# TAdeJong/pyGPA

Hardware: AMD Instinct MI355X
Metric: Mpixels/s displacement-field extraction (3 peaks, 4096^2 img) + achieved HBM GB/s (higher is better)
Workload: dtype f32; 1 GPU; 4096x4096 synthetic hex moire, 3 Bragg peaks x 16 k-vectors, sigma=10, weighted DCT-PCG unwrap kmax=10, image resident in HBM, u downloaded to pinned host memory inside the step (BASELINE.json configs[2]); x_planes=12, d2h_of_u=included, overlapped with the next step (copy stream), images_in_flight=1

## Files before the change

### pygpa_amd/csrc/gpa_api.hip

```cpp
#include "gpa_plan.h"

static thread_local std::string g_err;
int gpa_fail(int code, const std::string& msg) {
  g_err = msg;
  return code;
}
namespace gpa {
static const char* const kOptNames[OPT_COUNT] = {
    "PBS_FULLBAND", "SERIAL_UNWRAP", "NO_WORKER", "NO_KSPLIT", "NO_COMPACT", "NO_SHARED",
    "NO_PAIR", "PBS_E8", "TRI_SMALL", "TRI_Q", "NO_MR", "MR_FORCE_BLUESTEIN", "NO_ROWPQ", "COLSOLVE", "NO_LAT",
    "F32_EPS_FLOOR", "COLSTREAM_CHUNK", "NO_ROWHALF", "PAIR_MAXSIDE", "ROWHALF_MINLG", "NO_PQDCT",
    "NO_REORDER", "NO_RAW", "NO_TILEFUSE", "NO_ROWPERS", "NO_LFTILE", "LF_ALL_ROUNDS", "DFT_ENGINE", "GAUSS_FFT_MINR", "NO_GAUSS2D", "NO_DFT_HALF", "F32_STALL", "PBS_LDS_PAD", "NO_SHARED_PHASES", "PA_STAG", "PA_STAG_TICKS", "PA_ROT"};
static OptVal g_opts[OPT_COUNT];
static std::once_flag g_opts_once;
static void opt_assign(OptVal& o, const char* value) {
  o.set = value != nullptr;
  o.num = value ? atof(value) : 0.0;
  memset(o.str, 0, sizeof(o.str));
  if (value) strncpy(o.str, value, sizeof(o.str) - 1);
}
static void opts_from_env() {
  for (int k = 0; k < OPT_COUNT; ++k) opt_assign(g_opts[k], getenv((std::string("GPA_") + kOptNames[k]).c_str()));
}
const OptVal& opt(OptKey k) {
  std::call_once(g_opts_once, opts_from_env);
  return g_opts[k];
}
}

Axis make_axis(int n) {
  Axis a;
  a.n = n;
  int lg = 0;
  while ((1 << lg) < n) ++lg;
  if ((1 << lg) == n) {
    a.padded = false;
  } else {
    lg = 0;
    while ((1 << lg) < 2 * n - 1) ++lg;
    a.padded = true;
  }
  if (lg < 6) {
    lg = 6;
    a.padded = ((1 << lg) != n);
  }
  a.lg = lg;
  a.L = 1 << lg;
  a.extL = a.padded ? n - 1 : 0;
  a.extR = 0;
  return a;
}

Axis compact_axis(const Axis& full, int E) {
  if (!full.padded || E >= (full.n - 1) / 2) return full;
  int lg = 6;
  while ((1 << lg) < full.n + 2 * E) ++lg;
  if (lg >= full.lg) return full;
  Axis a = full;
  a.lg = lg;
  a.L = 1 << lg;
  a.extL = a.extR = E;
  return a;
}

int upload_real_table(gpa_plan* p, void* dst, const std::vector<double>& v) {
  if (p->dtype == GPA_F32) HIP_TRY(upload_as<float>(dst, v, p->stream));
  else HIP_TRY(upload_as<double>(dst, v, p->stream));
  return GPA_OK;
}

int dmalloc(gpa_plan* p, void** ptr, size_t bytes) {
  if (bytes == 0) bytes = 16;
  hipError_t e = hipMalloc(ptr, bytes);
  if (e != hipSuccess)
    return fail(GPA_ERR_HIP, std::string("hipMalloc(") + std::to_string(bytes) + "): " + hipGetErrorString(e));
  p->ws_bytes += bytes;
  return GPA_OK;
}
int plan_build(gpa_plan* p) {
  HIP_TRY(hipSetDevice(p->device));
  HIP_TRY(hipStreamCreateWithFlags(&p->stream, hipStreamNonBlocking));
  HIP_TRY(hipEventCreate(&p->ev0));
  HIP_TRY(hipEventCreate(&p->ev1));
  for (auto& e : p->stage_ev) HIP_TRY(hipEventCreate(&e));
  const size_t npx = (size_t)p->n0 * p->n1;
  const int B = p->max_batch;
  for (int ax = 0; ax < 2; ++ax) {
    const Axis& a = ax == 0 ? p->ax0 : p->ax1;
    std::vector<double> t((size_t)2 * a.L);
    for (int k = 0; k < a.L; ++k) {
      t[2 * k] = cos(-2.0 * M_PI * k / a.L);
      t[2 * k + 1] = sin(-2.0 * M_PI * k / a.L);
    }
    void** dst = ax == 0 ? &p->tw0 : &p->tw1;
    TRY(dmalloc(p, dst, (size_t)a.L * p->csz));
    TRY(upload_real_table(p, *dst, t));
  }
  TRY(dmalloc(p, &p->Hx, (size_t)p->ax0.L * p->csz));
  TRY(dmalloc(p, &p->Hy, (size_t)p->ax1.L * p->csz));
  p->tbuf_planes = B < 4 ? B : 4;
  TRY(dmalloc(p, &p->Tbuf, (size_t)p->tbuf_planes * npx * p->csz));
  TRY(dmalloc(p, &p->tb.cxb, (size_t)B * std::max(p->ax0.L / 16, 256) * p->csz));
  TRY(dmalloc(p, &p->tb.sx, (size_t)B * 16 * p->csz));
  TRY(dmalloc(p, &p->tb.wxw, (size_t)B * p->csz));
  TRY(dmalloc(p, &p->tb.wxr, (size_t)B * p->csz));
  TRY(dmalloc(p, &p->tb.cyb, (size_t)B * std::max(p->ax1.L / 16, 256) * p->csz));
  TRY(dmalloc(p, &p->tb.sy, (size_t)B * 16 * p->csz));
  TRY(dmalloc(p, &p->tb.wyw, (size_t)B * p->csz));
  TRY(dmalloc(p, &p->tb.wyr, (size_t)B * p->csz));
  TRY(dmalloc(p, (void**)&p->tb.planeof, (size_t)B * sizeof(int)));
  TRY(dmalloc(p, (void**)&p->d_pw, (size_t)B * sizeof(double)));
  TRY(dmalloc(p, &p->tb.dx, (size_t)B * p->n0 * p->csz));
  TRY(dmalloc(p, &p->tb.dy, (size_t)B * p->n1 * p->csz));
  TRY(dmalloc(p, (void**)&p->d_kl, (size_t)B * 2 * sizeof(double)));
  TRY(dmalloc(p, (void**)&p->d_kr, (size_t)B * 2 * sizeof(double)));
  HIP_TRY(hipHostMalloc((void**)&p->h_k, ((size_t)B * 6 + 32) * sizeof(double)));
  HIP_TRY(hipHostMalloc((void**)&p->h_iters, 8 * sizeof(int)));
  TRY(dmalloc(p, &p->d_image, npx * p->rsz));
  TRY(dmalloc(p, &p->d_mean, 16));
  TRY(dmalloc(p, &p->d_tile_mean, 16));
  TRY(dmalloc(p, (void**)&p->d_scratch, 16384 * sizeof(double)));
  TRY(dmalloc(p, &p->d_aux0, (size_t)p->n0 * 2 * sizeof(double)));
  TRY(dmalloc(p, &p->d_aux1, (size_t)p->n1 * 2 * sizeof(double)));
  p->max_peaks = B < 8 ? B : 8;
  TRY(dmalloc(p, &p->d_lockin, (size_t)p->max_peaks * npx * p->csz));
  TRY(dmalloc(p, (void**)&p->d_kidx, (size_t)p->max_peaks * npx * sizeof(int32_t)));
  TRY(dmalloc(p, &p->d_dudx, 2 * npx * p->rsz));
  TRY(dmalloc(p, &p->d_dudy, 2 * npx * p->rsz));
  TRY(dmalloc(p, &p->d_wnorm, npx * p->rsz));
  TRY(dmalloc(p, &p->d_u, 2 * npx * p->rsz));
  TRY(dmalloc(p, (void**)&p->d_kmat, (size_t)p->max_peaks * 2 * sizeof(double)));
  if (!p->spectral_only) {
    size_t before = 0;
    hipError_t e = unwrap_workspace_create(p->dtype, p->n0, p->n1, p->stream, &p->uw, &before);
    if (e != hipSuccess) return fail(GPA_ERR_HIP, std::string("unwrap workspace: ") + hipGetErrorString(e));
    p->ws_bytes += before;
  }
  return GPA_OK;
}


int upload_twiddles(gpa_plan* p, void* dst, int L) {
  std::vector<double> t((size_t)2 * L);
  for (int k = 0; k < L; ++k) {
    t[2 * k] = cos(-2.0 * M_PI * k / L);
    t[2 * k + 1] = sin(-2.0 * M_PI * k / L);
  }
  return upload_real_table(p, dst, t);
}

extern "C" {

int gpa_version(void) { return 100; }

int gpa_set_option(const char* name, const char* value) {
  if (!name) return fail(GPA_ERR_ARG, "gpa_set_option: null name");
  if (strncmp(name, "GPA_", 4) == 0) name += 4;
  (void)opt(OPT_NO_LAT);
  for (int k = 0; k < OPT_COUNT; ++k)
    if (strcmp(name, kOptNames[k]) == 0) {
      opt_assign(g_opts[k], value);
      return GPA_OK;
    }
  return fail(GPA_ERR_ARG, std::string("gpa_set_option: unknown option ") + name);
}
// ... 177 lines not shown
```

### pygpa_amd/csrc/gpa_internal.h

```cpp
#pragma once
#include <hip/hip_runtime.h>
#include <stdint.h>

#include "gpa_fft.h"
#include "gpa_mrfft.h"

namespace gpa {

struct KernelProfiler {
  struct Rec { const char* name; hipEvent_t a, b; };
  static constexpr int MAXREC = 4096;
  Rec rec[MAXREC];
  int n = 0;
  hipEvent_t pool[2 * MAXREC];
  int npool = 0;
};
extern thread_local KernelProfiler* g_kprof;
struct ProfScope {
  hipStream_t s;
  KernelProfiler::Rec* r = nullptr;
  ProfScope(const char* name, hipStream_t stream) : s(stream) {
    KernelProfiler* k = g_kprof;
    if (!k || k->n >= KernelProfiler::MAXREC) return;
    for (int j = 0; j < 2; ++j)
      if (k->npool < 2 * (k->n + 1)) { if (hipEventCreate(&k->pool[k->npool]) != hipSuccess) return; ++k->npool; }
    r = &k->rec[k->n];
    r->name = name;
    r->a = k->pool[2 * k->n];
    r->b = k->pool[2 * k->n + 1];
    ++k->n;
    (void)hipEventRecord(r->a, s);
  }
  ~ProfScope() { if (r) (void)hipEventRecord(r->b, s); }
};
#if defined(__HIPCC__)
__device__ __forceinline__ int xcd_tile(int b, int grid) {
  const int base = grid >> 3, rem = grid & 7, x = b & 7, idx = b >> 3;
  return x * base + (x < rem ? x : rem) + idx;
}
#endif

inline hipError_t set_dynamic_lds_once(const void* kern, int bytes, unsigned& done) {
  int dev = 0;
  (void)hipGetDevice(&dev);
  const unsigned bit = 1u << (dev & 31);
  if (done & bit) return hipSuccess;
  hipError_t e = hipFuncSetAttribute(kern, hipFuncAttributeMaxDynamicSharedMemorySize, bytes);
  if (e == hipSuccess) done |= bit;
  return e;
}

inline int device_cus() {
  static int n[32] = {};
  int dev = 0;
  (void)hipGetDevice(&dev);
  int& slot = n[dev & 31];
  if (!slot) {
    int cus = 0;
    if (hipDeviceGetAttribute(&cus, hipDeviceAttributeMultiprocessorCount, dev) != hipSuccess || cus <= 0) cus = 256;
    slot = cus;
  }
  return slot;
}

enum OptKey {
  OPT_PBS_FULLBAND, OPT_SERIAL_UNWRAP, OPT_NO_WORKER, OPT_NO_KSPLIT, OPT_NO_COMPACT, OPT_NO_SHARED,
  OPT_NO_PAIR, OPT_PBS_E8, OPT_TRI_SMALL, OPT_TRI_Q, OPT_NO_MR, OPT_MR_FORCE_BLUESTEIN, OPT_NO_ROWPQ,
  OPT_COLSOLVE, OPT_NO_LAT, OPT_F32_EPS_FLOOR, OPT_COLSTREAM_CHUNK, OPT_NO_ROWHALF, OPT_PAIR_MAXSIDE, OPT_ROWHALF_MINLG, OPT_NO_PQDCT,
  OPT_NO_REORDER, OPT_NO_RAW, OPT_NO_TILEFUSE, OPT_NO_ROWPERS, OPT_NO_LFTILE, OPT_LF_ALL_ROUNDS, OPT_DFT_ENGINE, OPT_GAUSS_FFT_MINR, OPT_NO_GAUSS2D, OPT_NO_DFT_HALF, OPT_F32_STALL, OPT_PBS_LDS_PAD, OPT_NO_SHARED_PHASES, OPT_PA_STAG, OPT_PA_STAG_TICKS, OPT_PA_ROT, OPT_COUNT
};
struct OptVal {
  bool set;
  double num;
  char str[24];
};
const OptVal& opt(OptKey k);
inline bool opt_set(OptKey k) { return opt(k).set; }

#define GPA_PROF_CAT2(a, b) a##b
#define GPA_PROF_CAT(a, b) GPA_PROF_CAT2(a, b)
#define GPA_PROF(name, stream) ::gpa::ProfScope GPA_PROF_CAT(_gpa_prof_, __LINE__)(name, stream)

struct Axis {
  int n;
  int lg;
  int L;
  bool padded;
  int extL, extR;
};
inline int axis_tpf(const Axis& a) { return a.L / 16; }

GPA_HD int axis_src(int m, int n, int L, bool padded, int extL, int extR) {
  if (!padded) return m;
  if (m < n) return m;
  if (m < n + extR) return m - n;
  if (m >= L - extL) return m - L + n;
  return -1;
}

struct SweepTables {
  void* cxb;
  void* sx;
  void* wxw;
  void* wxr;
  void* cyb;
  void* sy;
  void* wyw;
  void* wyr;
  void* dx;
  void* dy;
  int* planeof;
};

hipError_t launch_tables(int dtype, const Axis& a0, const Axis& a1, const double* kl,
                         const double* kr, int B, const double* pw, int Bx, const SweepTables& tb,
                         hipStream_t s);
hipError_t launch_mean(int dtype, const void* image, size_t count, double* scratch,
                       void* mean_out, hipStream_t s, int nimg = 1);
hipError_t launch_passA(int dtype, const Axis& a0, int n1, const void* image, const void* mean,
                        const SweepTables& tb, const void* Hx, const void* tw0, void* Tbuf,
                        int Bx, hipStream_t s, int nimg = 1);
hipError_t launch_passB(int dtype, const Axis& a1, int n0, const void* Tbuf, const void* Hy,
                        const void* tw1, const SweepTables& tb, int P, int K, bool select,
                        void* out, int32_t* kidx, hipStream_t s, int nimg = 1, int Bx = 0);
hipError_t launch_passB_ext(int dtype, const Axis& a1, int n0, const void* Tbuf, const void* Hy, const void* tw1,
                            const SweepTables& tb, int K, int mode, void* out, int32_t* kidx, const uint8_t* gate,
                            void* psi, hipStream_t s, int P = 1);
hipError_t launch_passB_split(int dtype, const Axis& a1, int n0, const void* Tbuf, const void* Hy, const void* tw1,
                              const SweepTables& tb, int P, int K, int ksplit, void* part, int32_t* pidx, void* out,
                              int32_t* kidx, hipStream_t s);
hipError_t launch_phasegrad(int dtype, const void* psi, int K, const int32_t* kidx, int n0, int n1, const double* kl,
                            const double* kr, int mode, void* grad, hipStream_t s, const double* ystep = nullptr, int P = 1);
int passA_cols(int dtype, int lg);
int spec_index_rt(int lg, int tid, int reg, int elems = 16);

hipError_t launch_reconstruct(int dtype, const void* lockin, const double* kmat ,
                              int P, int n0, int n1, int border, void* dudx, void* dudy,
                              void* wnorm, hipStream_t s, const double* ystep = nullptr );

hipError_t launch_reconstruct_tile(int dtype, const void* lockin, const double* kmat, int P, int n0, int n1, int border,
                                   int i0, int j0, int t0, int t1, void* const dx[2], size_t dx_pitch, void* const dy[2],
                                   size_t dy_pitch, void* const wn[2], size_t wn_pitch, hipStream_t s,
                                   const double* ystep = nullptr);
hipError_t launch_reconstruct_setup(int dtype, const void* lockin, const double* kmat, int P, int n0, int n1,
                                    int border, void* wnorm, void* r0, void* r1, double* part0, double* part1,
                                    int* nparts, hipStream_t s, int nimg = 1, size_t rstride = 0, size_t pstride = 0,
                                    const double* ystep = nullptr );

hipError_t launch_prediff(int dtype, const void* grads, const void* w, const double* kmat, int P, int n0, int n1,
                          void* dudx, void* dudy, void* wnorm, hipStream_t s);

hipError_t launch_wlstsq(int dtype, const void* b, const void* w, const double* kmat, int P, size_t npx,
                         void* out, hipStream_t s);

hipError_t launch_jacobian(int dtype, const void* grads, const void* w, const double* kmat, int P, size_t npx,
                           double nmperpixel, const double* dks , void* J, hipStream_t s);
hipError_t launch_cabs(int dtype, const void* z, size_t count, void* out, hipStream_t s);
hipError_t launch_props(int dtype, const void* jac, size_t npx, int add_identity, double refangle, double refscale,
                        int diff, void* out, hipStream_t s);

int huber_sums_offset();
hipError_t launch_huber_moments(int dtype, const void* img, int n0, int n1, const double* coef, double cx, double cy,
                                double sx, double sy, double* scratch, hipStream_t s);

constexpr int PEAK_PARTS = 1024;
bool gauss2d_small_ok(int R);
hipError_t launch_gauss2d_small(int dtype, const void* in, void* out, int n0, int n1, const double* w, int R,
                                const void* minuend, hipStream_t s);
hipError_t launch_gauss1d(int dtype, const void* in, void* out, int n0, int n1, int axis, const double* w, int R,
                          const void* minuend, hipStream_t s);
hipError_t launch_localmax(int dtype, const void* smooth, int n0, int n1, double rel, double* part, double* thr,
                           int max_out, int* count, int32_t* coords, void* vals, hipStream_t s);

hipError_t launch_deconv_pack(int dtype, const void* data, int m0, int m1, int pad, void* Z, hipStream_t s);
hipError_t launch_deconv_filter(int dtype, void* Z, int n0, int n1, const double* gx, const double* gy, double balance,
                                hipStream_t s);
hipError_t launch_deconv_unpack(int dtype, const void* Z, int m0, int m1, int pad, void* out, hipStream_t s);

hipError_t launch_tile_sums(int dtype, const void* wins, size_t win_stride, size_t pitch, const int* rects_dev, int ntiles,
                            int max_rows, double* part, double* out, hipStream_t s);
int tile_sums_bands(int max_rows);
hipError_t launch_set_mean(int dtype, const double* sum, double scale, void* mean_out, hipStream_t s);
hipError_t launch_copy_fields(int dtype, const void* const* src, void* const* dst, const size_t* src_pitch,
                              const size_t* dst_pitch, const int* rows, const int* cols, int nf, hipStream_t s);
hipError_t launch_stitch(int dtype, const void* tiles, size_t slot_stride, size_t field_stride, size_t tile_pitch,
                         const int* table_dev, int ntiles, int t0, int t1, int nf, void* const* dst, const size_t* dst_pitch,
                         const int* dst_rows, const int* dst_cols, hipStream_t s);

struct WarpWs {
  void* buf = nullptr;
  size_t cap = 0;
  void* taps = nullptr;
  int taps_dtype = -1;
  size_t* counted = nullptr;
};
void warp_ws_free(WarpWs* ws);
hipError_t warp_reserve_undistort(int dtype, int n0, int n1, WarpWs* ws, hipStream_t s);
hipError_t warp_invert_u(int dtype, const void* d_u, int n0, int n1, double scale, int iters, int edge, int shift,
                         void* d_out, hipStream_t s, int mode, int nan_last, WarpWs* ws, const int* rects = nullptr, int nrect = 0);
hipError_t warp_image(int dtype, const void* d_img, const void* d_uinv, int n0, int n1, void* d_out, hipStream_t s, WarpWs* ws,
                      const int* rects = nullptr, int nrect = 0);
hipError_t spline_coef_constant_f64(const double* d_in, int n0, int n1, double* d_tmp, double* d_out, hipStream_t s, WarpWs* ws);

struct UcellGeom {
  double ks[4], kinv[4], rmin[2], z;
  int rs0, rs1;
};
struct UcellWs {
  void* buf = nullptr;
  size_t cap = 0;
  WarpWs spline{};
  void* stage = nullptr;
  size_t stage_cap = 0;
  size_t* counted = nullptr;
};
void ucell_ws_free(UcellWs* ws);
hipError_t ucell_stage(UcellWs* ws, size_t bytes, hipStream_t s, void** out);
constexpr int UCELL_MAX_FRAMES = 65535;
constexpr long long UCELL_MAX_BINS = 1LL << 24;
hipError_t ucell_average(int dtype, const void* d_images, int B, const void* d_u, int n0, int n1, const UcellGeom& g,
                         double* d_res, double* d_weights, hipStream_t s, UcellWs* ws);
hipError_t ucell_expand(int dtype, const double* d_cell, const UcellGeom& g, double z2, const void* d_u, int n0, int n1,
// ... 4 lines not shown
```

### pygpa_amd/csrc/gpa_passb_shared.hip

```cpp
#include <stdlib.h>

#include "gpa_internal.h"
#include "gpa_passb_shared.h"

namespace gpa {

template <class T> struct MfmaVec;
template <> struct MfmaVec<float> { typedef float type __attribute__((ext_vector_type(4))); };
template <> struct MfmaVec<double> { typedef double type __attribute__((ext_vector_type(4))); };

__device__ __forceinline__ MfmaVec<float>::type mfma16(float a, float b, MfmaVec<float>::type c) {
  return __builtin_amdgcn_mfma_f32_16x16x4f32(a, b, c, 0, 0, 0);
}
__device__ __forceinline__ MfmaVec<double>::type mfma16(double a, double b, MfmaVec<double>::type c) {
  return __builtin_amdgcn_mfma_f64_16x16x4f64(a, b, c, 0, 0, 0);
}
template <class T> __device__ __forceinline__ int mfma_row(int kq, int r) {
  if constexpr (sizeof(T) == 8) return kq + 4 * r;
  else return 4 * kq + r;
}

template <class T> struct upair { T u, v; };

#ifndef GPA_PBS_NOFIX
#define GPA_PBS_NOFIX 0
#endif
#ifndef GPA_PBS_EXECSTORE
#define GPA_PBS_EXECSTORE 0
#endif
#ifndef GPA_PBS_NOSTORE
#define GPA_PBS_NOSTORE 0
#endif
#ifndef GPA_PBS_WAVESKIP
#define GPA_PBS_WAVESKIP 1
#endif
#ifndef GPA_PBS_NTLOAD
#define GPA_PBS_NTLOAD 1
#endif

template <class T, int TPF, int EE>
__device__ __forceinline__ void load_gb(T (&h)[EE], const T* gbrow, int tid) {
  using gscalar = const __attribute__((address_space(1))) T;
  gscalar* gb = (gscalar*)gbrow;
#pragma unroll
  for (int i = 0; i < EE; ++i) h[i] = gb[i * TPF + tid];
}
template <class T> __device__ __forceinline__ cpx<T> load_cpx(__amdgpu_buffer_rsrc_t r, int voff, int soff, int aux = 16);
__device__ __forceinline__ cpx<float> load_once(const cpx<float>* p) {
  typedef float v2f_t __attribute__((ext_vector_type(2)));
  const v2f_t d = __builtin_nontemporal_load(reinterpret_cast<const v2f_t*>(p));
  return {d.x, d.y};
}
__device__ __forceinline__ cpx<double> load_once(const cpx<double>* p) {
  typedef double v2d_t __attribute__((ext_vector_type(2)));
  const v2d_t d = __builtin_nontemporal_load(reinterpret_cast<const v2d_t*>(p));
  return {d.x, d.y};
}

typedef int v2i_t __attribute__((ext_vector_type(2)));
typedef int v4i_t __attribute__((ext_vector_type(4)));
__device__ __forceinline__ void store_cpx(cpx<double> v, __amdgpu_buffer_rsrc_t r, int voff, int soff);
__device__ __forceinline__ void store_cpx(cpx<float> v, __amdgpu_buffer_rsrc_t r, int voff, int soff) {
  v2i_t d = {__float_as_int(v.x), __float_as_int(v.y)};
  __builtin_amdgcn_raw_buffer_store_b64(d, r, voff, soff, 0);
}
template <> __device__ __forceinline__ cpx<float> load_cpx<float>(__amdgpu_buffer_rsrc_t r, int voff, int soff, int aux) {
  v2i_t d = aux == 16 ? __builtin_amdgcn_raw_buffer_load_b64(r, voff, soff, 16) : aux == 2 ? __builtin_amdgcn_raw_buffer_load_b64(r, voff, soff, 2) : __builtin_amdgcn_raw_buffer_load_b64(r, voff, soff, 0);
  return {__int_as_float(d.x), __int_as_float(d.y)};
}
template <> __device__ __forceinline__ cpx<double> load_cpx<double>(__amdgpu_buffer_rsrc_t r, int voff, int soff, int aux) {
  v4i_t d = aux == 16 ? __builtin_amdgcn_raw_buffer_load_b128(r, voff, soff, 16) : aux == 2 ? __builtin_amdgcn_raw_buffer_load_b128(r, voff, soff, 2) : __builtin_amdgcn_raw_buffer_load_b128(r, voff, soff, 0);
  const long long a = ((long long)(unsigned)d.x) | ((long long)d.y << 32), b = ((long long)(unsigned)d.z) | ((long long)d.w << 32);
  return {__longlong_as_double(a), __longlong_as_double(b)};
}
__device__ __forceinline__ void store_pair(cpx<float> a, cpx<float> b, __amdgpu_buffer_rsrc_t r, int voff, int soff) {
  v4i_t d = {__float_as_int(a.x), __float_as_int(a.y), __float_as_int(b.x), __float_as_int(b.y)};
  __builtin_amdgcn_raw_buffer_store_b128(d, r, voff, soff, 0);
}
__device__ __forceinline__ void store_pair(cpx<double> a, cpx<double> b, __amdgpu_buffer_rsrc_t r, int voff, int soff) {
  store_cpx(a, r, voff, soff);
  store_cpx(b, r, voff + 16, soff);
}
__device__ __forceinline__ void store_cpx(cpx<double> v, __amdgpu_buffer_rsrc_t r, int voff, int soff) {
  const long long a = __double_as_longlong(v.x), b = __double_as_longlong(v.y);
  v4i_t d = {(int)a, (int)(a >> 32), (int)b, (int)(b >> 32)};
  __builtin_amdgcn_raw_buffer_store_b128(d, r, voff, soff, 0);
}

template <class T, int LG, int EE = 16>
struct PassBSGeom {
  using F = WgFFT<T, LG, EE>;
  static_assert(F::P == 3 || F::P == 4, "three- or four-pass transforms");
  static constexpr int TPF = F::TPF;
  static_assert(TPF >= 64, "a row needs whole wavefronts");
#ifndef GPA_PBS_MINTHREADS
#define GPA_PBS_MINTHREADS 128
#endif
  static constexpr int NF = TPF >= GPA_PBS_MINTHREADS ? 1 : GPA_PBS_MINTHREADS / TPF;
  static constexpr int THREADS = NF * TPF;
  static constexpr int NW = TPF / 64;
  static constexpr int NC = PassBSharedNC<T>::value;
  static constexpr int LOGNC = NC == 4 ? 2 : 1;
  static constexpr bool STAGE = sizeof(T) == 4;
#ifndef GPA_PBS_TWL
#define GPA_PBS_TWL 1
#endif
  static constexpr bool TWL = GPA_PBS_TWL && F::P == 3;
  static constexpr int T1 = TWL ? F::P1_SETS * 6 : 0;
  static constexpr int SV = sizeof(T) == 4 ? 4 : 2;
  __host__ __device__ static size_t row_elems(int Epad) {
    const size_t ES = (size_t)Epad + 4;
    return (size_t)F::LDS_ELEMS + SV * ES + 2 * NC * ES + (STAGE ? 3 * NC * ES : 0);
  }
  __host__ __device__ static size_t lds_bytes(int Epad) {
    return (NF * row_elems(Epad) + T1) * sizeof(cpx<T>) + (2 * (size_t)Epad + 16) * sizeof(T);
  }
};

#ifndef GPA_PBS_F32_WAVES
#define GPA_PBS_F32_WAVES 3
#endif
#ifndef GPA_PBS_PAD_WAVES
#define GPA_PBS_PAD_WAVES 3
#endif
#ifndef GPA_PBS_F64_WAVES
#define GPA_PBS_F64_WAVES 2
#endif

#ifndef GPA_PBS_E8_WAVES
#define GPA_PBS_E8_WAVES 4
#endif
#ifndef GPA_PBS_E8_F64_WAVES
#define GPA_PBS_E8_F64_WAVES 2
#endif
#ifndef GPA_PBS_L13_WAVES
#define GPA_PBS_L13_WAVES 3
#endif
template <class T, int LG, bool PADDED, int EE, int NBL, bool PSI = false>
__global__ __launch_bounds__((PassBSGeom<T, LG, EE>::THREADS),
                             (EE == 8 ? (sizeof(T) == 8 ? GPA_PBS_E8_F64_WAVES : GPA_PBS_E8_WAVES)
                                      : (sizeof(T) == 8 ? GPA_PBS_F64_WAVES : (LG >= 13 ? GPA_PBS_L13_WAVES : (PADDED ? GPA_PBS_PAD_WAVES : GPA_PBS_F32_WAVES))))) void passB_shared_kernel(
    const cpx<T>* __restrict__ Tin, int n0, int n1, const T* __restrict__ Gb, const cpx<T>* __restrict__ twtab,
    const int* __restrict__ planeof, const int* __restrict__ order, const int* __restrict__ desc, const cpx<T>* __restrict__ pre_g,
    const cpx<T>* __restrict__ psi, const T* __restrict__ gtab, const cpx<T>* __restrict__ dx,
    const cpx<T>* __restrict__ dyc, const cpx<T>* __restrict__ rot16, int K, int E, int Epad, cpx<T>* out,
    int32_t* kidx, int P, int Bx, int raw, T* __restrict__ psi_out) {
  using F = WgFFT<T, LG, EE>;
  using G = PassBSGeom<T, LG, EE>;
  using V4 = typename MfmaVec<T>::type;
  constexpr int TPF = F::TPF, L = F::L, NC = G::NC;
  constexpr bool STAGE = G::STAGE;
  extern __shared__ __attribute__((aligned(16))) char smem[];
  const int tid = threadIdx.x % TPF, f = __builtin_amdgcn_readfirstlane(threadIdx.x / TPF);
  cpx<T>* lds = reinterpret_cast<cpx<T>*>(smem) + (size_t)f * G::row_elems(Epad);
  upair<T>* strip = reinterpret_cast<upair<T>*>(lds + F::LDS_ELEMS);
  const int ES = Epad + 4;
  cpx<T>* fixb = lds + F::LDS_ELEMS + G::SV * ES;
  cpx<T>* pre_l = fixb + 2 * NC * ES;
  cpx<T>* psi_l = pre_l + NC * ES;
  cpx<T>* t1 = reinterpret_cast<cpx<T>*>(smem) + (size_t)G::NF * G::row_elems(Epad);
  T* glds = reinterpret_cast<T*>(t1 + G::T1);
  const int row = blockIdx.x * G::NF + f;
  const bool valid = row < n0;
  const int rr = valid ? row : 0;
  const int p = blockIdx.y, pt = p % P, img = p / P;
  const int lane = threadIdx.x & 63, wrow = tid >> 6;

  for (int i = threadIdx.x; i < 2 * Epad + 16; i += G::THREADS) glds[i] = gtab[i];
#ifndef GPA_PBS_TWREG_F32
#define GPA_PBS_TWREG_F32 1
#endif
  constexpr bool TWLK = G::TWL && !(GPA_PBS_TWREG_F32 && sizeof(T) == 4 && !PADDED);
  typename std::conditional<TWLK, typename F::TwiddlesP1Lds, typename F::Twiddles>::type tw;
  if constexpr (TWLK) {
    F::fill_pass1_table(t1, twtab, threadIdx.x, G::THREADS);
    __syncthreads();
    F::load_twiddles(tw, twtab, tid, t1);
  } else {
    F::load_twiddles(tw, twtab, tid);
  }

  T ab[EE];
#pragma unroll
  for (int i = 0; i < EE; ++i) ab[i] = T(0);
  const size_t obase = ((size_t)p * n0 + rr) * n1;
  const __amdgpu_buffer_rsrc_t orow = __builtin_amdgcn_make_buffer_rsrc((void*)(out + obase), 0, n1 * (int)sizeof(cpx<T>), 0x00020000);
  const __amdgpu_buffer_rsrc_t krow = __builtin_amdgcn_make_buffer_rsrc((void*)(kidx ? kidx + obase : nullptr), 0, kidx ? n1 * 4 : 0, 0x00020000);
  constexpr int OOB = (int)0x80000000;
  const int iA = PADDED ? (n1 - E) / TPF : EE - 1, iB = PADDED ? (n1 - 1) / TPF : EE - 1;

  cpx<T> X[NBL];
  T h[NBL];
  const cpx<T> rot = rot16[pt * EE + (tid & (EE - 1))];
  const cpx<T> rot_tail = rot16[pt * EE + ((n1 - 1 - (tid < E ? tid : 0)) & (EE - 1))];
#ifndef GPA_PBS_PREFETCH_F64
#define GPA_PBS_PREFETCH_F64 0
#endif
#ifndef GPA_PBS_PREFETCH_F32
#define GPA_PBS_PREFETCH_F32 1
#endif
  constexpr bool PREFETCH = NBL < EE && (sizeof(T) == 8 ? GPA_PBS_PREFETCH_F64 : GPA_PBS_PREFETCH_F32);
  for (int k = 0; k < K; ++k) {
    const int b = pt * K + k;
    const int ob = order[b];
    const int d = desc[b];
    if (d & 1) {
      const cpx<T>* src = Tin + (((size_t)img * Bx + planeof[ob]) * n0 + rr) * n1;
      const cpx<T> cs0 = dx[(size_t)ob * n0 + rr];
      const cpx<T> cs = cmul(cs0, rot);
      cpx<T> tail = {T(0), T(0)};
      if (tid < E) tail = src[n1 - 1 - tid];
      cpx<T> XX[EE];
      if constexpr (PADDED) {
        const __amdgpu_buffer_rsrc_t srow = __builtin_amdgcn_make_buffer_rsrc((void*)src, 0, n1 * (int)sizeof(cpx<T>), 0x00020000);
#pragma unroll
        for (int i = 0; i < EE; ++i)
          XX[i] = cmul(load_cpx<T>(srow, (tid + TPF * i) * (int)sizeof(cpx<T>), 0, GPA_PBS_NTLOAD ? 2 : 0), cs);
      } else {
#pragma unroll
        for (int i = 0; i < EE; ++i) XX[i] = cmul(GPA_PBS_NTLOAD ? load_once(src + tid + TPF * i) : src[tid + TPF * i], cs);
      }
      if (tid < Epad) {
        const bool in = tid < E;
        const cpx<T> s0 = in ? XX[0] : cpx<T>{T(0), T(0)};
        const cpx<T> s1 = in ? cmul(tail, cmul(cs0, rot_tail)) : cpx<T>{T(0), T(0)};
        if constexpr (G::SV == 4) {
          strip[0 * ES + tid] = {s0.x, -s0.y};
          strip[1 * ES + tid] = {s0.y, s0.x};
          strip[2 * ES + tid] = {s1.x, s1.y};
          strip[3 * ES + tid] = {s1.y, -s1.x};
        } else {
          strip[0 * ES + tid] = {s0.x, s0.y};
          strip[1 * ES + tid] = {s1.x, s1.y};
        }
      }
      F::forward(XX, lds, tid, tw);
#pragma unroll
      for (int i = 0; i < NBL; ++i) X[i] = XX[i];
    }
    const int par = (d >> 7) & 1;
    cpx<T> y[EE];
    {
      if (!PREFETCH || k == 0) load_gb<T, TPF, NBL>(h, Gb + (size_t)b * (NBL * TPF), tid);
      if constexpr (STAGE) {
        if (d & 2) {
          const int nc = (d >> 4) & 7;
          for (int e = tid; e < NC * Epad; e += TPF) {
            const int c = e / Epad, j = e - c * Epad, cc = c < nc ? c : nc - 1;
            pre_l[c * ES + j] = pre_g[(size_t)(b + cc) * Epad + j];
            psi_l[(par * NC + c) * ES + j] = psi[(size_t)(b + cc) * Epad + j];
          }
        }
      }
#pragma unroll
      for (int i = 0; i < EE; ++i) {
        if (i < NBL) y[i] = {X[i < NBL ? i : 0].x * h[i < NBL ? i : 0], X[i < NBL ? i : 0].y * h[i < NBL ? i : 0]};
        else y[i] = {T(0), T(0)};
      }
    }
    cpx<T> psL = {T(0), T(0)}, psR = {T(0), T(0)};
    const int a0R = PADDED ? 0 : TPF - 1 - tid;
    if constexpr (!STAGE) {
      psL = psi[(size_t)b * Epad + (tid < E ? tid : 0)];
      psR = psi[(size_t)b * Epad + (a0R < E ? a0R : 0)];
    }
    F::template inv_phase<0>(y, lds, tid, tw);
    __syncthreads();
    if ((d & 2) && !GPA_PBS_NOFIX) {
      const int nc = (d >> 4) & 7;
      const int n = lane & 15, kq = lane >> 4;
      const int c = (n >> 1) & (NC - 1), end = (n >> (1 + G::LOGNC)) & 1, reim = n & 1;
      const cpx<T>* pre = STAGE ? pre_l + c * ES : pre_g + (size_t)(b + (c < nc ? c : nc - 1)) * Epad;
      const upair<T>* sp = strip + (G::SV == 4 ? end * 2 + reim : end) * ES;
      const bool swp = reim != 0;
      const T sgn = (end == 0) == swp ? T(1) : T(-1);
      const int Mt = (E + 15) >> 4;
      for (int mt = wrow; mt < Mt; mt += G::NW) {
        V4 acc0 = {T(0), T(0), T(0), T(0)}, acc1 = {T(0), T(0), T(0), T(0)};
        int ns = ((E - 16 * mt - 1) >> 2) + 1;
        if (ns > (Epad >> 2)) ns = Epad >> 2;
        const T* ga = glds + 16 * mt + (lane & 15) + kq + 1;
        for (int s = 0; s < ns; s += 4) {
          upair<T> q[4];
          cpx<T> pp[4];
          T av[4];
#pragma unroll
          for (int u = 0; u < 4; ++u) {
            int j = 4 * (s + u) + kq;
            j = j < Epad ? j : Epad - 1;
            q[u] = sp[j];
            if constexpr (G::SV == 2) q[u] = {swp ? q[u].v : q[u].u, sgn * (swp ? q[u].u : q[u].v)};
            pp[u] = pre[j];
            av[u] = ga[4 * (s + u)];
          }
#pragma unroll
          for (int u = 0; u < 4; ++u) {
            const T bv = q[u].u * pp[u].x + q[u].v * pp[u].y;
            if (u & 1) acc1 = mfma16(av[u], bv, acc1);
            else acc0 = mfma16(av[u], bv, acc0);
          }
        }
        if (n < 4 * NC) {
#pragma unroll
          for (int r = 0; r < 4; ++r) {
            const int a0 = 16 * mt + mfma_row<T>(kq, r);
            reinterpret_cast<T*>(fixb + (c * 2 + end) * ES + a0)[reim] = acc0[r] + acc1[r];
          }
        }
      }
    }
    F::template inv_phase<1>(y, lds, tid, tw);
    __syncthreads();
    F::template inv_phase<2>(y, lds, tid, tw);
    if constexpr (F::P == 4) {
      __syncthreads();
      F::template inv_phase<3>(y, lds, tid, tw);
    }
#if !GPA_PBS_NOFIX
    {
      const int c = (d >> 2) & 3;
      const cpx<T>* pl = psi_l + (par * NC + c) * ES;
      if (tid < E) {
        const cpx<T> fx = fixb[(c * 2 + 1) * ES + tid];
        if constexpr (STAGE) psL = pl[tid];
        const cpx<T> t = cmulc(fx, psL);
        y[0].x += t.x;
        y[0].y += t.y;
      }
      if constexpr (!PADDED) {
        if (a0R < E) {
          const cpx<T> fx = fixb[(c * 2 + 0) * ES + a0R];
          if constexpr (STAGE) psR = pl[a0R];
          const cpx<T> t = cmul(fx, psR);
          y[EE - 1].x += t.x;
          y[EE - 1].y += t.y;
        }
      } else {
        cpx<T> fA = {T(0), T(0)}, fB = {T(0), T(0)};
        {
          const int aA = n1 - 1 - (tid + TPF * iA), aB = aA - TPF;
          const bool inA = aA >= 0 && aA < E, inB = aB >= 0 && aB < E && iB != iA;
          const int qa = inA ? aA : 0, qb = inB ? aB : 0;
          const cpx<T> xa = fixb[(c * 2 + 0) * ES + qa], xb = fixb[(c * 2 + 0) * ES + qb];
          const cpx<T> pa = STAGE ? pl[qa] : psi[(size_t)b * Epad + qa], pb = STAGE ? pl[qb] : psi[(size_t)b * Epad + qb];
          const cpx<T> ta = cmul(xa, pa), tb2 = cmul(xb, pb);
          fA = {inA ? ta.x : T(0), inA ? ta.y : T(0)};
          fB = {inB ? tb2.x : T(0), inB ? tb2.y : T(0)};
        }
#pragma unroll
        for (int i = 0; i < EE; ++i) {
          if (i == iA) { y[i].x += fA.x; y[i].y += fA.y; }
          if (i == iB && iB != iA) { y[i].x += fB.x; y[i].y += fB.y; }
        }
      }
    }
#endif
    if constexpr (PREFETCH) {
      if (k + 1 < K) load_gb<T, TPF, NBL>(h, Gb + (size_t)(b + 1) * (NBL * TPF), tid);
    }
    const int kout = ob - pt * K;
    if constexpr (PSI) {
      if (valid) {
        T* prow = psi_out + ((size_t)(p * K + kout) * n0 + rr) * n1;
#pragma unroll
        for (int i = 0; i < EE; ++i) {
          const int yy = tid + TPF * i;
          if (!PADDED || yy < n1) prow[yy] = -atan2(y[i].y, y[i].x);
        }
      }
    }
#pragma unroll
    for (int i = 0; i < EE; ++i) {
      const int yy = tid + TPF * i;
      const T a = y[i].x * y[i].x + y[i].y * y[i].y;
      const bool win = a > ab[i];
      ab[i] = win ? a : ab[i];
#if GPA_PBS_WAVESKIP
      if (__builtin_amdgcn_ballot_w64(win) == 0) continue;
#endif
      const int woff = (win && valid) ? (PADDED ? yy : tid) * (int)sizeof(cpx<T>) : OOB;
      constexpr int SOFF = PADDED ? 0 : 1;
#if GPA_PBS_EXECSTORE
      if (woff != OOB) store_cpx(y[i], orow, woff, SOFF * i * TPF * (int)sizeof(cpx<T>));
      if (kidx && woff != OOB) __builtin_amdgcn_raw_buffer_store_b32(kout, krow, woff >> (sizeof(cpx<T>) == 8 ? 1 : 2), SOFF * i * TPF * 4, 0);
#elif !GPA_PBS_NOSTORE
      store_cpx(y[i], orow, woff, SOFF * i * TPF * (int)sizeof(cpx<T>));
      constexpr int SH = sizeof(cpx<T>) == 8 ? 1 : 2;
      if (kidx) __builtin_amdgcn_raw_buffer_store_b32(kout, krow, woff >> SH, SOFF * i * TPF * 4, 0);
#endif
    }
  }
  if (!valid) return;
  if (raw) {
#pragma unroll
    for (int i = 0; i < EE; ++i) {
      const int yy = tid + TPF * i;
      const bool never = !(ab[i] > T(0)) && (!PADDED || yy < n1);
      if (__builtin_amdgcn_ballot_w64(never) == 0) continue;
      if (never) {
        out[obase + yy] = cpx<T>{T(0), T(0)};
        if (kidx) kidx[obase + yy] = -1;
      }
    }
    return;
  }
  asm volatile("s_waitcnt vmcnt(0)" ::: "memory");
  const cpx<T>* dyp = dyc + (size_t)pt * n1;
  cpx<T> w[EE];
#pragma unroll
  for (int i = 0; i < EE; ++i) {
    const int yy = tid + TPF * i;
    w[i] = PADDED ? load_cpx<T>(orow, yy * (int)sizeof(cpx<T>), 0) : load_cpx<T>(orow, tid * (int)sizeof(cpx<T>), i * TPF * (int)sizeof(cpx<T>));
  }
#pragma unroll
  for (int i = 0; i < EE; ++i) {
    const int yy = tid + TPF * i;
    if (!PADDED || yy < n1) {
      cpx<T> v = {T(0), T(0)};
      if (ab[i] > T(0)) v = cmul(w[i], dyp[yy]);
      else if (kidx) kidx[obase + yy] = -1;
      out[obase + yy] = v;
    }
  }
}

template <class T>
__device__ __forceinline__ cpx<T> unit_phasor_s(double cycles) {
  double fr = cycles - rint(cycles);
  double s, c;
  sincospi(2.0 * fr, &s, &c);
  return {(T)c, (T)s};
}


template <class T, int LG, int EE>
__global__ __launch_bounds__(256) void shared_tables_kernel(const double* __restrict__ wys, const double* __restrict__ kr,
                                                           const int* __restrict__ shifts, const double* __restrict__ taps,
                                                           int Etab, int n1, int E, int Epad, int wrapped, int K, int nbl,
                                                           T* __restrict__ Gb, cpx<T>* __restrict__ psi,
                                                           cpx<T>* __restrict__ dyc, cpx<T>* __restrict__ pre,
                                                           cpx<T>* __restrict__ rot16) {
  using F = WgFFT<T, LG, EE>;
  constexpr int L = F::L, TPF = F::TPF;
  const int b = blockIdx.y;
  const int idx = blockIdx.x * 256 + threadIdx.x;
  const double wy = wys[b];
  if (idx < nbl * TPF) {
    const int i = idx / TPF, t = idx % TPF;
    const int kbin = F::spec_index(t, i);
    const double fq = wy + (double)kbin / (double)L;
    double acc = 0;
    for (int m = Etab; m >= 1; --m) {
      const double ph = fq * (double)m;
      acc += taps[m] * cospi(2.0 * (ph - rint(ph)));
    }
    Gb[(size_t)b * (nbl * TPF) + idx] = (T)((taps[0] + 2.0 * acc) / (double)L);
  }
  if (idx < Epad) {
    double ps, pc, qs, qc;
    const double c0 = -wy * (double)n1, c1 = wy * (double)(idx + 1);
    sincospi(2.0 * (c0 - rint(c0)), &ps, &pc);
    sincospi(2.0 * (c1 - rint(c1)), &qs, &qc);
    pc -= wrapped ? 1.0 : 0.0;
    cpx<T> v = {(T)(pc * qc - ps * qs), (T)(pc * qs + ps * qc)};
    if (idx >= E) v = {T(0), T(0)};
    psi[(size_t)b * Epad + idx] = v;
    pre[(size_t)b * Epad + idx] = unit_phasor_s<T>(wy * (double)idx);
  }
  if (b % K == 0) {
    const int p = b / K;
    const double sh = (double)shifts[p] / (double)EE;
    if (idx < n1) dyc[(size_t)p * n1 + idx] = unit_phasor_s<T>((kr[2 * b + 1] + sh) * (double)idx);
    if (idx < EE) rot16[p * EE + idx] = unit_phasor_s<T>(-sh * (double)idx);
  }
}

template <class T, int LG, int EE>
static hipError_t run_shared_tables(const Axis& a1, const double* wys, const double* kr, const int* shifts, const double* taps,
                                    int Etab, int E, int Epad, int B, int K, int nbl, const PassBSharedTables& st, hipStream_t s) {
  int len = a1.L > a1.n ? a1.L : a1.n;
  if (len < Epad) len = Epad;
  dim3 grid((len + 255) / 256, B);
  shared_tables_kernel<T, LG, EE><<<grid, 256, 0, s>>>(wys, kr, shifts, taps, Etab, a1.n, E, Epad, a1.padded ? 0 : 1, K, nbl,
                                                       (T*)st.Gb, (cpx<T>*)st.psi, (cpx<T>*)st.dyc, (cpx<T>*)st.pre,
                                                       (cpx<T>*)st.rot16);
  return hipGetLastError();
}

hipError_t launch_shared_tables(int dtype, const Axis& a1, const double* wys, const double* kr, const int* shifts,
                                const double* taps, int Etab, int E, int Epad, int B, int K, int nbl, const PassBSharedTables& st,
                                hipStream_t s, int elems) {
#ifdef GPA_PBS_BUILD_E8
#define CASE_T8(LG) CASE_T(LG, 8)
#else
#define CASE_T8(LG)
#endif
#define CASE_T(LG, EE)                                                                                                  \
  if (a1.lg == LG && elems == EE)                                                                                       \
    return dtype == 0 ? run_shared_tables<float, LG, EE>(a1, wys, kr, shifts, taps, Etab, E, Epad, B, K, nbl, st, s)    \
                      : run_shared_tables<double, LG, EE>(a1, wys, kr, shifts, taps, Etab, E, Epad, B, K, nbl, st, s);
  CASE_T(11, 16) CASE_T(12, 16) CASE_T(13, 16) CASE_T8(12)
#undef CASE_T
  return hipErrorInvalidValue;
}

template <class T, int LG, bool PADDED, int EE, int NBL, bool PSI = false>
static hipError_t run_passB_shared(const Axis& a1, int n0, const void* Tbuf, const void* tw1, const SweepTables& tb,
                                   const PassBSharedTables& st, int E, int Epad, int P, int K, void* out, int32_t* kidx,
                                   hipStream_t s, int nimg, int Bx, bool raw, void* psi_out = nullptr) {
  using G = PassBSGeom<T, LG, EE>;
  size_t lds = G::lds_bytes(Epad);
  if (lds > 160 * 1024 || E > G::TPF || Epad > G::TPF) return hipErrorInvalidValue;
  if (opt_set(OPT_PBS_LDS_PAD)) lds = std::min<size_t>(160 * 1024, lds + (size_t)opt(OPT_PBS_LDS_PAD).num);
  auto kern = passB_shared_kernel<T, LG, PADDED, EE, NBL, PSI>;
  static int lds_set[32] = {0};
  int dev = 0;
  (void)hipGetDevice(&dev);
  if (lds_set[dev & 31] < (int)lds) {
    hipError_t e = hipFuncSetAttribute(reinterpret_cast<const void*>(kern), hipFuncAttributeMaxDynamicSharedMemorySize, (int)lds);
    if (e != hipSuccess) return e;
    lds_set[dev & 31] = (int)lds;
  }
  dim3 grid((n0 + G::NF - 1) / G::NF, P * nimg);
  GPA_PROF(PSI ? "passB_shared_phases_kernel" : "passB_shared_kernel", s);
  kern<<<grid, G::THREADS, lds, s>>>((const cpx<T>*)Tbuf, n0, a1.n, (const T*)st.Gb, (const cpx<T>*)tw1, tb.planeof, st.order, st.desc,
                                     (const cpx<T>*)st.pre, (const cpx<T>*)st.psi, (const T*)st.gtab, (const cpx<T>*)tb.dx,
                                     (const cpx<T>*)st.dyc, (const cpx<T>*)st.rot16, K, E, Epad, (cpx<T>*)out, kidx, P, Bx, raw ? 1 : 0, (T*)psi_out);
  return hipGetLastError();
}

int passB_shared_elems(int dtype, const Axis& a1) {
  (void)dtype;
#ifdef GPA_PBS_BUILD_E8
  const bool e8 = opt_set(OPT_PBS_E8);
  return (a1.lg == 12 && e8) ? 8 : 16;
#else
  (void)a1;
  return 16;
#endif
}

bool passB_shared_supports(int dtype, const Axis& a1, int E) {
  if (a1.lg < 11 || a1.lg > (dtype == 0 ? 13 : 12)) return false;
  const int tpf = a1.L / 16;
  const int Epad = (E + 15) & ~15;
  if (E < 1 || Epad > tpf || 2 * E > a1.n) return false;
  if (a1.padded && a1.n + E > a1.L) return false;
  const size_t csz = dtype == 0 ? 8 : 16;
  const int nf = tpf >= GPA_PBS_MINTHREADS ? 1 : GPA_PBS_MINTHREADS / tpf, nc = dtype == 0 ? 4 : 2;
  const size_t ES = (size_t)Epad + 4;
  const size_t stage = dtype == 0 ? 3 * nc * ES : 0;
  const size_t lds = (nf * ((size_t)(a1.L + a1.L / 16) + (dtype == 0 ? 4 : 2) * ES + 2 * nc * ES + stage) + 16 * 6) * csz +
                     (2 * (size_t)Epad + 16) * (csz / 2);
  return lds <= 160 * 1024;
}

int passB_shared_nbl(int dtype, int need) {
  if (dtype == 0 && need <= 6) return 6;
  if (need <= 8) return 8;
  return 16;
}

hipError_t launch_passB_shared_phases(int dtype, const Axis& a1, int n0, const void* Tbuf, const void* tw1, const SweepTables& tb,
                                      const PassBSharedTables& st, int E, int Epad, int P, int K, void* out, int32_t* kidx,
                                      void* psi_out, hipStream_t s, int Bx, int elems, int nbl) {
  if (!psi_out || !kidx) return hipErrorInvalidValue;
#define CALL_P(T, LG, EE, NBL) \
  (a1.padded ? run_passB_shared<T, LG, true, EE, NBL, true>(a1, n0, Tbuf, tw1, tb, st, E, Epad, P, K, out, kidx, s, 1, Bx, false, psi_out) \
             : run_passB_shared<T, LG, false, EE, NBL, true>(a1, n0, Tbuf, tw1, tb, st, E, Epad, P, K, out, kidx, s, 1, Bx, false, psi_out))
#define CASE_P(LG, EE, NBL) \
  if (a1.lg == LG && elems == EE && nbl == NBL) return dtype == 0 ? CALL_P(float, LG, EE, NBL) : CALL_P(double, LG, EE, NBL);
#define CASE_PF32(LG, EE, NBL) \
  if (a1.lg == LG && elems == EE && nbl == NBL && dtype == 0) return CALL_P(float, LG, EE, NBL);
  CASE_PF32(11, 16, 6) CASE_PF32(12, 16, 6) CASE_PF32(13, 16, 6) CASE_PF32(13, 16, 8) CASE_PF32(13, 16, 16)
  CASE_P(11, 16, 8) CASE_P(12, 16, 8) CASE_P(11, 16, 16) CASE_P(12, 16, 16)
#undef CASE_PF32
#undef CASE_P
#undef CALL_P
  return hipErrorInvalidValue;
}

hipError_t launch_passB_shared(int dtype, const Axis& a1, int n0, const void* Tbuf, const void* tw1, const SweepTables& tb,
                               const PassBSharedTables& st, int E, int Epad, int P, int K, void* out, int32_t* kidx,
                               hipStream_t s, int nimg, int Bx, int elems, int nbl, bool raw) {
#define CALL_S(T, LG, EE, NBL) \
  (a1.padded ? run_passB_shared<T, LG, true, EE, NBL>(a1, n0, Tbuf, tw1, tb, st, E, Epad, P, K, out, kidx, s, nimg, Bx, raw) \
             : run_passB_shared<T, LG, false, EE, NBL>(a1, n0, Tbuf, tw1, tb, st, E, Epad, P, K, out, kidx, s, nimg, Bx, raw))
#define CASE_S(LG, EE, NBL) \
  if (a1.lg == LG && elems == EE && nbl == NBL) return dtype == 0 ? CALL_S(float, LG, EE, NBL) : CALL_S(double, LG, EE, NBL);
#define CASE_F32(LG, EE, NBL) \
  if (a1.lg == LG && elems == EE && nbl == NBL && dtype == 0) return CALL_S(float, LG, EE, NBL);
  CASE_F32(11, 16, 6) CASE_F32(12, 16, 6) CASE_F32(13, 16, 6) CASE_F32(13, 16, 8) CASE_F32(13, 16, 16)
  CASE_S(11, 16, 8) CASE_S(12, 16, 8) CASE_S(11, 16, 16) CASE_S(12, 16, 16)
#ifdef GPA_PBS_BUILD_E8
  CASE_S(12, 8, 8)
#endif
#undef CASE_F32
#undef CASE_S
#undef CALL_S
  return hipErrorInvalidValue;
}

}
```

Before: 3132 Mpixels/s.

## Compute first inverse FFT pass of passB_shared on matrix cores

For the f32, 4096-point, unpadded passB_shared kernel with six live band registers, the first radix-16 inverse FFT pass is replaced by 32x32x2 MFMA products of a cosine/sine weight matrix against the band-limited inputs. Lanes are exchanged with permlane32_swap and the results are written straight into LDS with stride 17. The intent is to move the butterfly arithmetic of the sparse first pass (only 6 of 16 inputs are nonzero) off the vector ALUs. The trade-off is a new LDS write pattern and MFMA latency, plus a hand-built twiddle layout whose index mapping must match the existing pass exactly. An environment option disables the path.

Result: slower. 3065 Mpixels/s (-2.1%).

```diff
diff --git a/pygpa_amd/csrc/gpa_api.hip b/pygpa_amd/csrc/gpa_api.hip
--- a/pygpa_amd/csrc/gpa_api.hip
+++ b/pygpa_amd/csrc/gpa_api.hip
@@ -10,7 +10,7 @@
     "PBS_FULLBAND", "SERIAL_UNWRAP", "NO_WORKER", "NO_KSPLIT", "NO_COMPACT", "NO_SHARED",
     "NO_PAIR", "PBS_E8", "TRI_SMALL", "TRI_Q", "NO_MR", "MR_FORCE_BLUESTEIN", "NO_ROWPQ", "COLSOLVE", "NO_LAT",
     "F32_EPS_FLOOR", "COLSTREAM_CHUNK", "NO_ROWHALF", "PAIR_MAXSIDE", "ROWHALF_MINLG", "NO_PQDCT",
-    "NO_REORDER", "NO_RAW", "NO_TILEFUSE", "NO_ROWPERS", "NO_LFTILE", "LF_ALL_ROUNDS", "DFT_ENGINE", "GAUSS_FFT_MINR", "NO_GAUSS2D", "NO_DFT_HALF", "F32_STALL", "PBS_LDS_PAD", "NO_SHARED_PHASES", "PA_STAG", "PA_STAG_TICKS", "PA_ROT"};
+    "NO_REORDER", "NO_RAW", "NO_TILEFUSE", "NO_ROWPERS", "NO_LFTILE", "LF_ALL_ROUNDS", "DFT_ENGINE", "GAUSS_FFT_MINR", "NO_GAUSS2D", "NO_DFT_HALF", "F32_STALL", "PBS_LDS_PAD", "NO_SHARED_PHASES", "PA_STAG", "PA_STAG_TICKS", "PA_ROT", "NO_PBS_MFMA"};
 static OptVal g_opts[OPT_COUNT];
 static std::once_flag g_opts_once;
 static void opt_assign(OptVal& o, const char* value) {
diff --git a/pygpa_amd/csrc/gpa_internal.h b/pygpa_amd/csrc/gpa_internal.h
--- a/pygpa_amd/csrc/gpa_internal.h
+++ b/pygpa_amd/csrc/gpa_internal.h
@@ -67,7 +67,7 @@
   OPT_PBS_FULLBAND, OPT_SERIAL_UNWRAP, OPT_NO_WORKER, OPT_NO_KSPLIT, OPT_NO_COMPACT, OPT_NO_SHARED,
   OPT_NO_PAIR, OPT_PBS_E8, OPT_TRI_SMALL, OPT_TRI_Q, OPT_NO_MR, OPT_MR_FORCE_BLUESTEIN, OPT_NO_ROWPQ,
   OPT_COLSOLVE, OPT_NO_LAT, OPT_F32_EPS_FLOOR, OPT_COLSTREAM_CHUNK, OPT_NO_ROWHALF, OPT_PAIR_MAXSIDE, OPT_ROWHALF_MINLG, OPT_NO_PQDCT,
-  OPT_NO_REORDER, OPT_NO_RAW, OPT_NO_TILEFUSE, OPT_NO_ROWPERS, OPT_NO_LFTILE, OPT_LF_ALL_ROUNDS, OPT_DFT_ENGINE, OPT_GAUSS_FFT_MINR, OPT_NO_GAUSS2D, OPT_NO_DFT_HALF, OPT_F32_STALL, OPT_PBS_LDS_PAD, OPT_NO_SHARED_PHASES, OPT_PA_STAG, OPT_PA_STAG_TICKS, OPT_PA_ROT, OPT_COUNT
+  OPT_NO_REORDER, OPT_NO_RAW, OPT_NO_TILEFUSE, OPT_NO_ROWPERS, OPT_NO_LFTILE, OPT_LF_ALL_ROUNDS, OPT_DFT_ENGINE, OPT_GAUSS_FFT_MINR, OPT_NO_GAUSS2D, OPT_NO_DFT_HALF, OPT_F32_STALL, OPT_PBS_LDS_PAD, OPT_NO_SHARED_PHASES, OPT_PA_STAG, OPT_PA_STAG_TICKS, OPT_PA_ROT, OPT_NO_PBS_MFMA, OPT_COUNT
 };
 struct OptVal {
   bool set;
diff --git a/pygpa_amd/csrc/gpa_passb_shared.hip b/pygpa_amd/csrc/gpa_passb_shared.hip
--- a/pygpa_amd/csrc/gpa_passb_shared.hip
+++ b/pygpa_amd/csrc/gpa_passb_shared.hip
@@ -21,6 +21,45 @@
 }
 
 template <class T> struct upair { T u, v; };
+
+typedef float v16f_t __attribute__((ext_vector_type(16)));
+__device__ const float kCos16[16] = {1.0f, (float)0.92387953251128673848, (float)0.70710678118654752440, (float)0.38268343236508978178,
+                                     0.0f, (float)-0.38268343236508978178, (float)-0.70710678118654752440, (float)-0.92387953251128673848,
+                                     -1.0f, (float)-0.92387953251128673848, (float)-0.70710678118654752440, (float)-0.38268343236508978178,
+                                     0.0f, (float)0.38268343236508978178, (float)0.70710678118654752440, (float)0.92387953251128673848};
+template <int NBL> struct InvPass0Mfma {
+  float w[NBL];
+  __device__ __forceinline__ void init(int lane) {
+    const int i = lane & 31, e = 2 * (i >> 2) + ((i >> 1) & 1), part = i & 1, k = lane >> 5;
+#pragma unroll
+    for (int s = 0; s < NBL; ++s) {
+      const int m = (e * s) & 15;
+      const float c = kCos16[m], sn = kCos16[(m + 12) & 15];
+      w[s] = part == 0 ? (k == 0 ? c : -sn) : (k == 0 ? sn : c);
+    }
+  }
+  __device__ __forceinline__ void run(const cpx<float> (&X)[NBL], const float (&h)[NBL], cpx<float>* lds, int col0, int lane) const {
+    v16f_t lo = {0, 0, 0, 0, 0, 0, 0, 0, 0, 0, 0, 0, 0, 0, 0, 0}, hi = lo;
+#pragma unroll
+    for (int s = 0; s < NBL; ++s) {
+      const auto r = __builtin_amdgcn_permlane32_swap(__float_as_uint(X[s].x * h[s]), __float_as_uint(X[s].y * h[s]), false, false);
+      lo = __builtin_amdgcn_mfma_f32_32x32x2f32(w[s], __uint_as_float(r[0]), lo, 0, 0, 0);
+      hi = __builtin_amdgcn_mfma_f32_32x32x2f32(w[s], __uint_as_float(r[1]), hi, 0, 0, 0);
+    }
+    cpx<float>* base = lds + 17 * (col0 + (lane & 31)) + 2 * (lane >> 5);
+#pragma unroll
+    for (int m = 0; m < 4; ++m) {
+      base[4 * m] = {lo[4 * m], lo[4 * m + 1]};
+      base[4 * m + 1] = {lo[4 * m + 2], lo[4 * m + 3]};
+    }
+    base += 17 * 32;
+#pragma unroll
+    for (int m = 0; m < 4; ++m) {
+      base[4 * m] = {hi[4 * m], hi[4 * m + 1]};
+      base[4 * m + 1] = {hi[4 * m + 2], hi[4 * m + 3]};
+    }
+  }
+};
 
 #ifndef GPA_PBS_NOFIX
 #define GPA_PBS_NOFIX 0
@@ -136,7 +175,7 @@
 #ifndef GPA_PBS_L13_WAVES
 #define GPA_PBS_L13_WAVES 3
 #endif
-template <class T, int LG, bool PADDED, int EE, int NBL, bool PSI = false>
+template <class T, int LG, bool PADDED, int EE, int NBL, bool PSI = false, bool MFMA0 = false>
 __global__ __launch_bounds__((PassBSGeom<T, LG, EE>::THREADS),
                              (EE == 8 ? (sizeof(T) == 8 ? GPA_PBS_E8_F64_WAVES : GPA_PBS_E8_WAVES)
                                       : (sizeof(T) == 8 ? GPA_PBS_F64_WAVES : (LG >= 13 ? GPA_PBS_L13_WAVES : (PADDED ? GPA_PBS_PAD_WAVES : GPA_PBS_F32_WAVES))))) void passB_shared_kernel(
@@ -150,6 +189,8 @@
   using V4 = typename MfmaVec<T>::type;
   constexpr int TPF = F::TPF, L = F::L, NC = G::NC;
   constexpr bool STAGE = G::STAGE;
+  static_assert(!MFMA0 || (sizeof(T) == 4 && EE == 16 && NBL == 6 && F::P == 3 && F::bits(F::P - 1) == 4),
+                "the matrix-core first inverse pass: f32, sixteen elements per thread, six live registers, radix-16 last pass");
   extern __shared__ __attribute__((aligned(16))) char smem[];
   const int tid = threadIdx.x % TPF, f = __builtin_amdgcn_readfirstlane(threadIdx.x / TPF);
   cpx<T>* lds = reinterpret_cast<cpx<T>*>(smem) + (size_t)f * G::row_elems(Epad);
@@ -180,6 +221,9 @@
     F::load_twiddles(tw, twtab, tid);
   }
 
+  InvPass0Mfma<MFMA0 ? NBL : 1> mf;
+  if constexpr (MFMA0) mf.init(lane);
+
   T ab[EE];
 #pragma unroll
   for (int i = 0; i < EE; ++i) ab[i] = T(0);
@@ -252,10 +296,12 @@
           }
         }
       }
-#pragma unroll
-      for (int i = 0; i < EE; ++i) {
-        if (i < NBL) y[i] = {X[i < NBL ? i : 0].x * h[i < NBL ? i : 0], X[i < NBL ? i : 0].y * h[i < NBL ? i : 0]};
-        else y[i] = {T(0), T(0)};
+      if constexpr (!MFMA0) {
+#pragma unroll
+        for (int i = 0; i < EE; ++i) {
+          if (i < NBL) y[i] = {X[i < NBL ? i : 0].x * h[i < NBL ? i : 0], X[i < NBL ? i : 0].y * h[i < NBL ? i : 0]};
+          else y[i] = {T(0), T(0)};
+        }
       }
     }
     cpx<T> psL = {T(0), T(0)}, psR = {T(0), T(0)};
@@ -264,7 +310,8 @@
       psL = psi[(size_t)b * Epad + (tid < E ? tid : 0)];
       psR = psi[(size_t)b * Epad + (a0R < E ? a0R : 0)];
     }
-    F::template inv_phase<0>(y, lds, tid, tw);
+    if constexpr (MFMA0) mf.run(X, h, lds, tid & ~63, lane);
+    else F::template inv_phase<0>(y, lds, tid, tw);
     __syncthreads();
     if ((d & 2) && !GPA_PBS_NOFIX) {
       const int nc = (d >> 4) & 7;
@@ -504,7 +551,7 @@
   return hipErrorInvalidValue;
 }
 
-template <class T, int LG, bool PADDED, int EE, int NBL, bool PSI = false>
+template <class T, int LG, bool PADDED, int EE, int NBL, bool PSI = false, bool MFMA0 = false>
 static hipError_t run_passB_shared(const Axis& a1, int n0, const void* Tbuf, const void* tw1, const SweepTables& tb,
                                    const PassBSharedTables& st, int E, int Epad, int P, int K, void* out, int32_t* kidx,
                                    hipStream_t s, int nimg, int Bx, bool raw, void* psi_out = nullptr) {
@@ -512,7 +559,7 @@
   size_t lds = G::lds_bytes(Epad);
   if (lds > 160 * 1024 || E > G::TPF || Epad > G::TPF) return hipErrorInvalidValue;
   if (opt_set(OPT_PBS_LDS_PAD)) lds = std::min<size_t>(160 * 1024, lds + (size_t)opt(OPT_PBS_LDS_PAD).num);
-  auto kern = passB_shared_kernel<T, LG, PADDED, EE, NBL, PSI>;
+  auto kern = passB_shared_kernel<T, LG, PADDED, EE, NBL, PSI, MFMA0>;
   static int lds_set[32] = {0};
   int dev = 0;
   (void)hipGetDevice(&dev);
@@ -559,6 +606,10 @@
   if (dtype == 0 && need <= 6) return 6;
   if (need <= 8) return 8;
   return 16;
+}
+
+static bool passB_shared_mfma0(int dtype, const Axis& a1, int elems, int nbl) {
+  return dtype == 0 && a1.lg == 12 && !a1.padded && elems == 16 && nbl == 6 && !opt_set(OPT_NO_PBS_MFMA);
 }
 
 hipError_t launch_passB_shared_phases(int dtype, const Axis& a1, int n0, const void* Tbuf, const void* tw1, const SweepTables& tb,
@@ -583,6 +634,8 @@
 hipError_t launch_passB_shared(int dtype, const Axis& a1, int n0, const void* Tbuf, const void* tw1, const SweepTables& tb,
                                const PassBSharedTables& st, int E, int Epad, int P, int K, void* out, int32_t* kidx,
                                hipStream_t s, int nimg, int Bx, int elems, int nbl, bool raw) {
+  if (passB_shared_mfma0(dtype, a1, elems, nbl))
+    return run_passB_shared<float, 12, false, 16, 6, false, true>(a1, n0, Tbuf, tw1, tb, st, E, Epad, P, K, out, kidx, s, nimg, Bx, raw);
 #define CALL_S(T, LG, EE, NBL) \
   (a1.padded ? run_passB_shared<T, LG, true, EE, NBL>(a1, n0, Tbuf, tw1, tb, st, E, Epad, P, K, out, kidx, s, nimg, Bx, raw) \
              : run_passB_shared<T, LG, false, EE, NBL>(a1, n0, Tbuf, tw1, tb, st, E, Epad, P, K, out, kidx, s, nimg, Bx, raw))
```
